# vfrantc/Bayesian-Enhancement-Model

Hardware: AMD Instinct MI355X
Metric: images/sec (whole node) CG_UNet N=8 Bayesian eval @256x256 (higher is better)
Workload: dtype f32

## Files before the change

bayesian-enhancement-model_amd/bem/modules.py:

```python
from __future__ import annotations

import math
from typing import Optional

import torch
import torch.nn as nn

from . import autograd as ag
from . import ops
from .bayes import BayesBank, Conv2dReparameterization, EvalSampleBank, Linear2dReparameterization, SampleCtx, sampling, set_module_paths
from .native import BemNativeError


def grad_mode(m: nn.Module) -> bool:
    return m.training and torch.is_grad_enabled()


def _need_cuda(x):
    if not x.is_cuda:
        raise BemNativeError("BEM modules run on the GPU through libbem_hip.so only (no CPU fallback); "
                             "move the model and input to a HIP device")


class LayerNorm2d(nn.LayerNorm):
# ... 131 lines not shown


class gdMlp(nn.Module):
    def __init__(self, in_features, hidden_features=None, out_features=None, act_layer=nn.GELU, drop=0.0, channels_first=False):
        super().__init__()
        out_features = out_features or in_features
        hidden_features = hidden_features or in_features
        self.project_in = PwConv2d(in_features, hidden_features * 2)
        self.dwconv = DwConv2d(hidden_features * 2)
        self.project_out = PwConv2d(hidden_features, out_features)
        self.act = act_layer()

    def fused_supported(self, C):
        return isinstance(self.project_in, PwConv2d) and isinstance(self.dwconv, DwConv2d) and isinstance(self.project_out, PwConv2d) \
            and ops.gdmlp_x6_supported(C, self.project_in.out_channels // 2)

    def forward_fused(self, x, norm: LayerNorm2d, pre=None):
        B, C = x.shape[0], x.shape[1]
        Hd = self.project_in.out_channels // 2
        if self.fused_supported(C):
            pi, dw, po = self.project_in, self.dwconv, self.project_out

            def prep():
                perm = ops.gate_interleave(Hd, pi.weight.device)
                bg = pi.bias.detach()[perm].contiguous() if pi.bias is not None else torch.zeros(2 * Hd, device=pi.weight.device)
                return (ops.pack_pw_weight(pi.weight.detach().reshape(2 * Hd, C)[perm].contiguous(), x6=True), bg,
                        ops.dw_gate_params10(dw.weight.detach(), None if dw.bias is None else dw.bias.detach(), Hd),
                        ops.pack_pw_weight(po.weight.detach().reshape(po.out_channels, Hd).contiguous(), x6=True),
                        None if po.bias is None else po.bias.detach().contiguous())
            Wg, bg, w10, Wo, bo = ops.derived(self).get("gdmlp_x6", [t for t in (pi.weight, pi.bias, dw.weight, dw.bias, po.weight, po.bias) if t is not None], prep)
            return ops.gdmlp_x6(x, norm.weight.detach(), norm.bias.detach(), norm.eps, Wg, bg, w10, Wo, bo, Hd, pre=pre)
        if pre is not None:
            raise BemNativeError("gdMlp: the SS2D tail can be folded into the one-kernel branch only")
        return self.chain(x, norm)[0]

    def chain(self, x, norm: LayerNorm2d):
        B = x.shape[0]
        t2 = ag.ln_pw(x, norm, self.project_in)
        w, b = self.dwconv.dw_weights(B)
        g = ops.dwconv3x3(t2, w, b, mode=2)
        Wp, b = self.project_out.gemm_weights(B)
        return ops.pw_gemm(g, Wp, ag.out_width(self.project_out), bias=b, res=x), t2, g


SS2D_MAX_D_STATE = 16


class SS2D(nn.Module):

    def __init__(self, d_model=96, d_state=16, ssm_ratio=2.0, dt_rank="auto", act_layer=nn.SiLU, d_conv=3,
                 conv_bias=True, dropout=0.0, bias=False, dt_min=0.001, dt_max=0.1, dt_init="random", dt_scale=1.0,
                 dt_init_floor=1e-4, initialize="v0", forward_type="v2", channel_first=False, **kwargs):
        super().__init__()
        if forward_type != "v05_noz" or not channel_first or d_conv != 3 or initialize != "v0":
            raise NotImplementedError("SS2D: only forward_type='v05_noz', channel_first, d_conv=3, init v0 are on the BEM path")
        N = int(d_state)
        if not 1 <= N <= SS2D_MAX_D_STATE:
            raise NotImplementedError(f"SS2D: d_state = {N}: the fused HIP scans take 1 <= d_state <= {SS2D_MAX_D_STATE}")
        d_inner = int(ssm_ratio * d_model)
        R = math.ceil(d_model / 16) if dt_rank == "auto" else dt_rank
        self.d_inner, self.dt_rank, self.d_state = d_inner, R, N
        self.in_proj = Linear2d(d_model, d_inner, bias=bias)
        self.act = act_layer()
        self.conv2d = DwConv2d(d_inner, bias=conv_bias)
        K = 4
        self.x_proj_weight = nn.Parameter(torch.stack([nn.Linear(d_inner, R + 2 * N, bias=False).weight.detach() for _ in range(K)], 0))
        self.out_proj = Linear2d(d_inner, d_model, bias=bias)
# ... 110 lines not shown
```

bayesian-enhancement-model_amd/bem/ops.py:

```python
from __future__ import annotations

import ctypes
import os
from inspect import signature as _signature
from functools import wraps as _wraps
from math import prod as _prod
from typing import Optional

import torch

from . import native
from .native import PwArgs, check, lib
from .tables import UIQM_WIDTH, lab_tables, niqe_gamma_table, niqe_resize_table, pil_resize_table, uiqm_resized_rows


_U64 = (1 << 64) - 1


def _stream():
    return ctypes.c_void_p(torch.cuda.current_stream().cuda_stream)


def _p(t: Optional[torch.Tensor]):
    return ctypes.c_void_p(0 if t is None else t.data_ptr())
# ... 575 lines not shown
    for n_, t in (("x", x), ("ln_w", ln_w), ("ln_b", ln_b), ("Wp_gate", Wp_gate), ("bias_gate", bias_gate), ("dw10", dw10), ("Wp_out", Wp_out)):
        _chk(t, n_)
    _chk(bias_out, "bias_out", optional=True)
    B, C, H, W = x.shape
    if not gdmlp_x6_supported(C, Hd):
        raise ValueError(f"gdmlp_x6: C = {C} (<= 80) / Hd = {Hd} (% 16) not supported")
    if tuple(dw10.shape) != (Hd, 10, 2):
        raise ValueError("gdmlp_x6: depthwise parameters must come from dw_gate_params10")
    if ln_w.numel() != C or ln_b.numel() != C or bias_gate.numel() != 2 * Hd or (bias_out is not None and bias_out.numel() != C):
        raise ValueError("gdmlp_x6: parameter shapes")
    _chk_packed1("gdmlp_x6", (("Wp_gate", Wp_gate, 2 * Hd, C), ("Wp_out", Wp_out, C, Hd)))
    _tile_plane_set("gdmlp_x6", C * H * W)
    if pre is not None:
        y0, y1, on_w, on_b, on_eps, Wp_op, b_op = pre
        for n_, t in (("y0", y0), ("y1", y1), ("on_w", on_w), ("on_b", on_b), ("Wp_outproj", Wp_op)):
            _chk(t, n_)
        _chk(b_op, "bias_outproj", optional=True)
        if not vss_back_supported(C, Hd, H * W):
            raise ValueError(f"gdmlp_x6 with pre: C = {C} (<= 48, % 8) with {C * H * W} elements per image (< {_TILE_NARROW}) not supported")
        if y0.shape != x.shape or y1.shape != x.shape or on_w.numel() != C or on_b.numel() != C or (b_op is not None and b_op.numel() != C):
            raise ValueError("gdmlp_x6 with pre: y0 / y1 must have the shape of x, out_norm and the out_proj bias C entries")
        _chk_packed1("gdmlp_x6", (("Wp_outproj", Wp_op, 32 * ((8 * ((C + 15) // 16) + 15) // 16), C),))
    out = torch.empty_like(x)
    if pre is not None:
        check(lib().bem_vss_back_x6_f32(_p(x), _p(ln_w), _p(ln_b), float(ln_eps), _p(Wp_gate), _p(bias_gate), _p(dw10), _p(Wp_out),
                                        _p(bias_out), _p(out), B, C, Hd, H, W, _p(y0), _p(y1), _p(on_w), _p(on_b), float(on_eps),
                                        _p(Wp_op), _p(b_op), _stream()), "gdmlp_x6")
        return out
    check(lib().bem_gdmlp_x6_f32(_p(x), _p(ln_w), _p(ln_b), float(ln_eps), _p(Wp_gate), _p(bias_gate), _p(dw10), _p(Wp_out),
                                 _p(bias_out), _p(out), B, C, Hd, H, W, _stream()), "gdmlp_x6")
    return out


def _dwconv3x3_cost(x, mode, **_):
    B, Cin, H, W = x.shape
    return 4.0 * B * H * W * (Cin + (Cin // 2 if mode == 2 else Cin)), 18.0 * B * Cin * H * W


@_bracket(_dwconv3x3_cost)
def dwconv3x3(x, w, bias=None, mode=0):
    _chk(x, "x"); _chk(w, "w"); _chk(bias, "bias", optional=True)
    B, Cin, H, W = x.shape
    Cout = Cin // 2 if mode == 2 else Cin
    per_b = w.dim() == 5
    Cw = w.shape[1] if per_b else w.shape[0]
    if Cw != Cin or tuple(w.shape[-3:]) != (1, 3, 3) or (per_b and w.shape[0] != B):
        raise ValueError(f"dwconv3x3: weight {tuple(w.shape)} vs input channels {Cin}")
    bb = 0
    if bias is not None:
        if bias.shape[-1] != Cin:
            raise ValueError("dwconv3x3: bias shape")
        bb = Cin if (bias.dim() == 2 and bias.shape[0] == B and B > 1) else 0
        if bias.dim() == 2 and bias.shape[0] not in (1, B):
            raise ValueError("dwconv3x3: bias batch")
    out = torch.empty(B, Cout, H, W, device=x.device, dtype=x.dtype)
    check(lib().bem_dwconv3x3_f32(_p(x), _p(w), (Cin * 9 if per_b else 0), _p(bias), bb, _p(out), B, Cout, H, W, mode,
                                  _stream()), "dwconv3x3")
    return out


USE_CONV_MFMA = True
USE_CONV_X6 = True


class ConvWeight:

    def __init__(self, w, input_grad=None):
        self.w, self._x6, self._f32, self._grad = w, None, None, input_grad

    def x6(self):
        if self._x6 is None:
            w = self.w
            self._x6 = pack_pw_weight(w.permute(2, 3, 0, 1).reshape(w.shape[2] * w.shape[3], w.shape[0], w.shape[1]).contiguous(), x6=True)
        return self._x6

    def f32(self):
        if self._f32 is None:
            self._f32 = pack_pw_weight(self.w.reshape(self.w.shape[0], -1).contiguous(), x6=False)
        return self._f32

    def input_grad(self):
        if self._grad is None:
            self._grad = ConvWeight(self.w.flip(2, 3).transpose(0, 1).contiguous())
        return self._grad


_CONV_FORMS = {1: ("rows", ConvWeight.x6), 2: ("taps", ConvWeight.x6), 3: ("mfma", ConvWeight.f32), 4: ("direct", lambda cw: cw.w)}
_CONV_ROUTES = {}


def _conv_out_hw(H, W, KH, KW, stride, pad, dilation=1):
    return (H + 2 * pad - dilation * (KH - 1) - 1) // stride + 1, (W + 2 * pad - dilation * (KW - 1) - 1) // stride + 1


def _conv2d_cost(x, w, stride, pad, res1, res2, dilation, **_):
# ... 12 lines not shown
    B, Ct, H, W = x.shape
    Cout, Cin, KH, KW = w.shape
    c0 = 0
    if cin_slice is not None:
        c0, cs = cin_slice
        if cs != Cin or c0 + Cin > Ct:
            raise ValueError("conv2d: channel slice out of range")
    elif Ct != Cin:
        raise ValueError(f"conv2d: input has {Ct} channels, weight expects {Cin}")
    if bias is not None and bias.shape != (Cout,):
        raise ValueError("conv2d: bias shape")
    if res1_rep < 1 or (res1_rep != 1 and res1 is None):
        raise ValueError("conv2d: res1_rep must be >= 1 and needs res1")
    oshape = (B, Cout) + _conv_out_hw(H, W, KH, KW, stride, pad, dilation)
    for n, r, shp in (("res1", res1, (B // res1_rep if B % res1_rep == 0 else -1,) + oshape[1:]), ("res2", res2, oshape)):
        if r is not None and tuple(r.shape) != shp:
            raise ValueError(f"conv2d: {n} shape")
    xs = _pslice(x, c0)
    key = (Cout, Cin, KH, KW, H, W, xs[1], stride, pad, dilation, USE_CONV_X6, USE_CONV_MFMA, (xs[0].value or 0) & 15,
           None if res1 is None else res1.data_ptr() & 15, None if res2 is None else res2.data_ptr() & 15)
    form = _CONV_ROUTES.get(key) or _CONV_ROUTES.setdefault(key, lib().bem_conv2d_route(
        *xs, _p(res1), _p(res2), None, Cin, H, W, Cout, KH, KW, stride, pad, dilation, USE_CONV_X6 | 2 * USE_CONV_MFMA))
    if form == 0:
        raise native.BemNativeError(lib().bem_last_error().decode())
    return form, cw, xs, oshape


def conv2d_route(x, w, stride=1, pad=1, res1=None, res2=None, cin_slice=None, dilation=1, res1_rep=1):
    return _CONV_FORMS[_conv2d_ask(x, w, None, stride, pad, res1, res2, cin_slice, dilation, res1_rep)[0]][0]


@_bracket(_conv2d_cost)
def conv2d(x, w, bias=None, stride=1, pad=1, relu=False, res1=None, res2=None, cin_slice=None, dilation=1, res1_rep=1):
    res1_rep = int(res1_rep)
    form, cw, xs, oshape = _conv2d_ask(x, w, bias, stride, pad, res1, res2, cin_slice, dilation, res1_rep)
    out = torch.empty(oshape, device=x.device, dtype=x.dtype)
    name, operand = _CONV_FORMS[form]
    (B, _, H, W), (Cout, Cin, KH, KW) = x.shape, cw.w.shape
    check(lib().bem_conv2d_f32(form, *xs, _p(operand(cw)), _p(bias), _p(res1), _p(res2), _p(out), B, Cin, H, W, Cout, KH, KW, stride, pad, dilation,
                               int(relu), res1_rep, _stream()), "conv2d " + name)
    return out


def quat_dwt(x, c0=0):
    _chk(x, "x")
    B, Ct, H, W = x.shape
    if c0 + 3 > Ct or H % 2 or W % 2:
        raise ValueError("quat_dwt: needs 3 channels and even H, W")
    out = torch.empty(B, 32, H // 2, W // 2, device=x.device, dtype=x.dtype)
    check(lib().bem_quat_dwt_f32(*_pslice(x, c0), _p(out), B, H, W, _stream()), "quat_dwt")
    return out


def cond_dwt(conds, s):
    _chk(conds, "conds")
    s = int(s)
    R, C, H, W = conds.shape
    if C != 3 or s < 1 or (H * s) % 2 or (W * s) % 2:
        raise ValueError("cond_dwt: needs 3 channels and even enlarged H, W")
    out = torch.empty(R, 32, H * s // 2, W * s // 2, device=conds.device, dtype=conds.dtype)
    check(lib().bem_cond_dwt_f32(_p(conds), _p(out), R, H, W, s, _stream()), "cond_dwt")
    return out


def dwt(x):
    _chk(x, "x")
    B, C, H, W = x.shape
# ... 1343 lines not shown
```

bayesian-enhancement-model_amd/csrc/gdmlp_x6.hip:

```cpp
#include "bem_common.h"
#include "x6_tile.h"

namespace {

struct GdX {
    const float* x; const float* ln_w; const float* ln_b; float ln_eps;
    const u32x4* Wpi;
    const u32x4* Wpo;
    const float* bgi;
    const float* dw10;
    int C, Hd, H, W, NCH, tx;
};

struct GdPre {
    const float* y0; const float* y1; const float* on_w; const float* on_b; float on_eps;
    const u32x4* Wop;
    const float* bop; float bopmul;
};

template <typename OFF>
__device__ __forceinline__ float at_byte(const float* base, OFF byte) {
    return *reinterpret_cast<const float*>(reinterpret_cast<const char*>(base) + byte);
}
template <typename OFF>
__device__ __forceinline__ void put_byte(float* base, OFF byte, float v) {
    *reinterpret_cast<float*>(reinterpret_cast<char*>(base) + byte) = v;
}

constexpr int GD_GS = 20;
constexpr bool GD_LO_PERSIST = true;

__device__ __forceinline__ float gelu_gate1(float a, float b) {
    const float t = __builtin_amdgcn_rcpf(fmaf(0.3275911f * 0.70710678118654752440f, fabsf(a), 1.f));
    float p = fmaf(1.061405429f, t, -1.453152027f);
    p = fmaf(p, t, 1.421413741f);
    p = fmaf(p, t, -0.284496736f);
    p = fmaf(p, t, 0.254829592f);
    const float e = __builtin_amdgcn_exp2f(a * a * -0.72134752044448170368f);
    const float r = fmaf(-(p * t), e, 1.f);
    const float h = 0.5f * a;
    return fmaf(h, copysignf(r, a), h) * b;
}

template <int KBM, int MTO, int WOB, bool PL2, bool PRE, typename OFF = uint32_t>
__device__ __forceinline__ void gdmlp_x6_tile(const GdX& k, const GdPre& pre, const float* __restrict__ bpo, float bomul, float* __restrict__ out) {
    constexpr int NPI = 3 * KBM, NPO = 3 * MTO;
    __shared__ __attribute__((aligned(16))) f32x2 T[16 * XT_TS];
    __shared__ __attribute__((aligned(16))) float G[128 * GD_GS];
    __shared__ __attribute__((aligned(16))) u32x4 Wis[2][NPI * 64];
    __shared__ __attribute__((aligned(16))) u32x4 Wos[WOB][NPO * 64];
    __shared__ __attribute__((aligned(16))) f32x2 Bss[2][16];
    __shared__ __attribute__((aligned(16))) f32x2 DWs[2][16 * 10];
    const int lane = threadIdx.x & 63, wave = __builtin_amdgcn_readfirstlane(threadIdx.x >> 6), kh = lane >> 5, n = lane & 31;
    const int b = blockIdx.z;
    int y0, x0;
    tile_origin(k.tx, y0, x0);
    const int L = k.H * k.W;
    const float* xb = k.x + (int64_t)b * k.C * L;

    const uint32_t voff = 16 * lane;
    const uint32_t wi_lds = lds_addr(Wis), wo_lds = lds_addr(Wos), bs_lds = lds_addr(Bss), dw_lds = lds_addr(DWs);
    auto dma_in = [&](int ji, int buf) {
#pragma unroll
        for (int t = 0; t < (NPI + 3) / 4; ++t) {
            const int p = wave + 4 * t;
            if (p < NPI) glds16(k.Wpi + ((int64_t)ji * NPI + p) * 64, voff, wi_lds + (buf * NPI + p) * 1024);
        }
        if (wave == (NPI & 3)) {
            const float* src = k.dw10 + (int64_t)ji * 320;
            glds16(src, voff, dw_lds + buf * 1280);
            if (lane < 16) glds16(src + 256, voff, dw_lds + buf * 1280 + 1024);
        }
        if (wave == ((NPI + 1) & 3) && lane < 8) glds16(k.bgi + (int64_t)ji * 32, voff, bs_lds + buf * 128);
    };
    auto dma_out = [&](int jo, int buf) {
// ... 487 lines not shown
```

include/bem_hip.h:

```cpp
#ifndef BEM_HIP_H
#define BEM_HIP_H

#include <stdint.h>

#ifdef __cplusplus
extern "C" {
#endif

#define BEM_OK 0
#define BEM_ERR_INVALID 1
#define BEM_ERR_LAUNCH 2

const char* bem_last_error(void);
int bem_abi_version(void);


int bem_selective_scan_fwd_f32(const float* u, const float* delta, const float* A, const float* Bm,
                               const float* Cm, const float* D, const float* delta_bias, float* out,
                               int batch, int dim, int L, int dstate, int ngroups, int delta_softplus,
                               void* stream);

int bem_selective_scan_fwd_in16(const void* u, const void* delta, const float* A, const void* Bm, const void* Cm, const float* D,
                                const float* delta_bias, float* out, int in_dtype, int batch, int dim, int L, int dstate,
                                int ngroups, int delta_softplus, void* stream);
// ... 40 lines not shown
    float* out; int out_mode; int Win;
    int B; int M; int K; int L;
} bem_pw_args;
int bem_pack_pw_weight_f32(const float* W, float* Wp, int nsets, int M, int K, void* stream);
int64_t bem_pw_packed_elems(int M, int K);

int bem_pw_gemm_x6_f32(const bem_pw_args* a, void* stream);
int bem_pack_pw_weight_x6(const float* W, float* Wp, int nsets, int M, int K, void* stream);
int bem_pack_pw_weight_x6_strided(const float* W, float* Wp, int nsets, int M, int K, int64_t set_stride, int64_t row_stride,
                                  int64_t col_stride, void* stream);
int bem_pack_pw_weight_x6_jobs(const void* jobs, const void* blks, int nblk, float* arena, void* stream);
int64_t bem_pw_x6_packed_elems(int M, int K);
int bem_bnn_sample_pack_x6(const float* mu, const float* rho, const float* eps, float* Wp, int nsets, int M, int K,
                           uint64_t seed, uint64_t stream_id, const uint64_t* stream_add, int sigma_given,
                           void* stream);
int bem_upfuse_x6_f32(const float* f, const float* skip, const float* Wc_packed, const float* Wf2_packed, const float* bias, float* out,
                      int B, int Cin, int h, int w, void* stream);

int bem_dwconv3x3_f32(const float* x, const float* w, int64_t w_bstride, const float* bias,
                      int64_t bias_bstride, float* out, int B, int Cout, int H, int W, int mode, void* stream);

#define BEM_CONV_ROWS 1
#define BEM_CONV_TAPS 2
#define BEM_CONV_MFMA 3
#define BEM_CONV_DIRECT 4
int bem_conv2d_f32(int form, const float* x, int64_t x_bstride, const float* w, const float* bias, const float* res1, const float* res2,
                   float* out, int B, int Cin, int H, int W, int Cout, int KH, int KW, int stride, int pad, int dilation, int relu,
                   int res1_rep, void* stream);

#define BEM_CONV_ALLOW_X6 1
#define BEM_CONV_ALLOW_MFMA 2
int bem_conv2d_route(const float* x, int64_t x_bstride, const float* res1, const float* res2, const float* out, int Cin, int H, int W,
                     int Cout, int KH, int KW, int stride, int pad, int dilation, int allow);

int bem_quat_dwt_f32(const float* rgb, int64_t x_bstride, float* out, int B, int H, int W, void* stream);
int bem_cond_dwt_f32(const float* cond, float* out, int R, int H, int W, int s, void* stream);
int bem_dwt_f32(const float* x, float* out, int B, int C, int H, int W, void* stream);
int bem_iwt_f32(const float* x, float* out, int B, int C4, int H, int W, void* stream);
int bem_iwt_hamilton_f32(const float* q1w, const float* q2w, float* out, int B, int h, int w, void* stream);
int bem_hamilton_f32(const float* q, float* out, int B, int H, int W, void* stream);

int bem_hamilton_full_f32(const float* q1, const float* q2, float* out, int B, int H, int W, void* stream);

int bem_attn_stats_f64(const float* f1, const float* f2, double* stats, int B, int L, void* stream);
int bem_attn_fold_f32(const double* stats, const float* attn_w ,
                      const float* fuse_w , const float* fuse_b ,
                      float* W_out , float* bias_out , int B, int L,
                      void* stream);
int bem_attn_fold_drop_f32(const double* stats, const float* attn_w, const float* fuse_w, const float* fuse_b,
                           const float* mask_or_null, float p, uint64_t seed, uint64_t stream_id,
                           float* W_out, float* bias_out, int B, int L, void* stream);

int bem_transpose_planes_f32(const float* src, int64_t src_bstride, float* dst, int64_t dst_bstride,
                             int nbatch, int ppb, int H, int W, void* stream);
int bem_copy_channels_f32(const float* src, int64_t src_bstride, float* dst, int64_t dst_bstride,
                          int B, int C, int L, void* stream);
int bem_copy_channels_rep_f32(const float* src, int64_t src_bstride, float* dst, int64_t dst_bstride, int B, int C, int L, int rep,
                              void* stream);
int bem_add_channels_f32(const float* src, int64_t src_bstride, float* dst, int64_t dst_bstride,
                         int B, int C, int L, void* stream);
int bem_bilinear_up_f32(const float* src, int64_t src_bstride, float* dst, int64_t dst_bstride,
                        int B, int C, int H, int W, int s, void* stream);
int bem_space_to_depth_f32(const float* x, float* out, int B, int C, int H, int W, void* stream);
int bem_pixel_shuffle2_f32(const float* x, float* out, int B, int C, int H, int W, void* stream);

int bem_bnn_ebank_sample_f32(const void* segs, const void* blks, int nblk, float* arena, uint64_t seed, uint64_t stream_base, void* stream);
// ... 22 lines not shown
int bem_candidate_finalize_f32(const float* pred, const float* target, float* final_out, float* psnr, double* ws,
                               int Bn, int samples_per_image, int Hp, int Wp, int h, int w, int gt_mean,
                               void* stream);

int bem_ssim_f32(const float* pred, const float* target, float* ssim, double* ws, int Bn, int samples_per_image, int h, int w, void* stream);

int bem_select_scores_f32(const float* cand, const float* s1, const float* s2, float weight, int rule, int* best, float* best_s1,
                          float* best_s2, float* best_img, int B, int N, int64_t chw, void* stream);

int bem_niqe_f32(const float* final, const double* mu_pris, const double* cov_pris, const double* window, const double* gam_tab, int ntab,
                 const float* rs_wh, const int* rs_ih, int kh, const float* rs_ww, const int* rs_iw, int kw, double* scores, void* ws,
                 int64_t ws_bytes, int Bn, int h, int w, void* stream);
int64_t bem_niqe_ws_bytes(int Bn, int h, int w);

int bem_uiqm_uciqe_f32(const float* final, const int* lab_tab, const int* rs_bh, const int* rs_kh, int kh, const int* rs_bv, const int* rs_kv,
                       int kv, double* uiqm, double* uciqe, void* ws, int64_t ws_bytes, int Bn, int h, int w, int Hr, void* stream);
int64_t bem_uiqm_ws_bytes(int Bn, int h, int w, int Hr);

int bem_mc_mean_f32(const float* pred, const float* target, float* out, double* ws, int B, int N, int Hp, int Wp, int h, int w,
                    int gt_mean, void* stream);

int bem_mc_accum_f32(const float* raw, const float* fin, float* sum, float* mean, float* m2, int B, int Nc, int n_done, int Hp, int Wp,
                     int h, int w, void* stream);

int bem_mc_finish_f32(const float* sum, const float* m2, const float* target, float* mc, float* std, double* std_mean, double* ws, int B,
                      int N, int h, int w, int gt_mean, void* stream);

int bem_select_merge_f32(const float* cand, const float* scores, int rule, int* best, float* best_score, float* best_img, int* pick, int B,
                         int Nc, int n_done, int64_t chw, void* stream);

int bem_gdmlp_x6_f32(const float* x, const float* ln_w, const float* ln_b, float ln_eps, const float* Wp_gate,
                     const float* bias_gate, const float* dw_gate10, const float* Wp_out,
                     const float* bias_out, float* out, int B, int C, int Hd, int H, int W, void* stream);

int bem_vss_back_x6_f32(const float* x, const float* ln_w, const float* ln_b, float ln_eps, const float* Wp_gate,
                        const float* bias_gate, const float* dw_gate10, const float* Wp_out,
                        const float* bias_out, float* out, int B, int C, int Hd, int H, int W,
                        const float* y0, const float* y1, const float* on_w, const float* on_b, float on_eps,
                        const float* Wp_outproj, const float* bias_outproj, void* stream);

int bem_ss2d_front_x6_f32(const float* x, const float* ln_w, const float* ln_b, float ln_eps, const float* Wp_in, const float* bias_in,
                          const float* dww, const float* dwb, const float* Wp_x, float* xc, float* xd, int B, int C, int Mx, int H, int W,
                          void* stream);


int bem_l1_loss_f32(const float* pred, const float* gt, float* dpred, float* loss, double* ws, int64_t n, float weight,
                    const float* gmul, void* stream);

int bem_ssim_loss_tile(void);
int64_t bem_ssim_loss_ws_elems(int64_t planes, int H, int W);
int bem_ssim_loss_f32(const float* pred, const float* gt, float* loss, float* coef, double* ws, int64_t planes, int H, int W,
                      float weight, void* stream);
int bem_ssim_loss_bwd_f32(const float* pred, const float* gt, const float* coef, float* dpred, int64_t planes, int H, int W,
                          float weight, const float* gmul, void* stream);

int bem_mse_loss_f32(const float* pred, const float* gt, float* dpred, float* loss, double* ws, int64_t n, float weight,
                     const float* gmul, void* stream);

int bem_pixstat_loss_chunk(void);
int64_t bem_pixstat_loss_ws_bytes(int64_t B, int64_t n1);
int bem_pixstat_loss_f32(const float* pred, const float* gt, float* out, double* rec, void* ws, int64_t B, int64_t n1, double a1,
                         double a3, double a5, double a6, void* stream);
int bem_pixstat_loss_bwd_f32(const float* pred, const float* gt, const double* rec, float* dpred, int64_t B, int64_t n1,
                             const float* gmul, void* stream);

int bem_iwt_hamilton_bwd_f32(const float* q1w, const float* q2w, const float* dout, float* dq1w, float* dq2w, int B, int h, int w,
// ... 124 lines not shown
```

bayesian-enhancement-model_amd/csrc/conv_x6.hip:

```cpp
#include "bem_common.h"
#include "conv_launch.h"
#include "scan_common.h"
#include "x6_common.h"

namespace {

struct CrX {
    const float* x; int64_t x_bs;
    const u32x4* Wp; const float* bias; const float* res1; const float* res2; float* out;
    int Cin, H, W, Ho, Wo, Cout, KB, MT, wo_shift, relu, mt_first, res1_rep;
};

typedef float f32x4v __attribute__((ext_vector_type(4)));

template <int MTW, int KS, int S>
__global__ __launch_bounds__(256, 2) void conv_rows_x6_kernel(CrX k) {
    constexpr int NPX = 4 / S;
    constexpr int NP = 3 * KS * MTW;
    __shared__ __attribute__((aligned(16))) u32x4 Ws[2][NP * 64];
    const int lane = threadIdx.x & 63, wave = __builtin_amdgcn_readfirstlane(threadIdx.x >> 6), kh = lane >> 5, n = lane & 31;
    const int b = blockIdx.z, mt0 = k.mt_first + blockIdx.y * MTW;
    const int Lo = k.Ho * k.Wo, Li = k.H * k.W;
    const int p0 = (xcd_tile(blockIdx.x, gridDim.x) * 4 + wave) * (32 * NPX);
    const int p = p0 + NPX * n;
    const bool live = p < Lo;
    const int pc = live ? p : 0;
    const int yo = pc >> k.wo_shift, xo = pc & (k.Wo - 1);
    const float lmask = xo == 0 ? 0.f : 1.f, rmask = xo == k.Wo - NPX ? 0.f : 1.f;
    const float* xb = k.x + (int64_t)b * k.x_bs;
    const uint32_t voff = 16 * lane, ws_lds = lds_addr(Ws);
    const int NS = KS * k.KB;

    auto dma_w = [&](int s, int buf) {
        const int kb = s / KS, r = s - kb * KS;
#pragma unroll
        for (int t = 0; t < (NP + 3) / 4; ++t) {
            const int pi = wave + 4 * t, kx = pi / (3 * MTW), m = (pi / 3) % MTW, li = pi % 3;
            if (pi < NP)
                glds16(k.Wp + ((((int64_t)(KS * r + kx) * k.MT + (mt0 + m)) * k.KB + kb) * 3 + li) * 64, voff, ws_lds + (buf * NP + pi) * 1024);
        }
    };
    auto load_x = [&](int s, f32x4v (&dst)[8], float& mk) {
        const int kb = min(s / KS, k.KB - 1), r = s - (s / KS) * KS;
// ... 42 lines not shown
                const u32x4* wp = Wc + (kx * MTW + m) * 192;
                const u32x4 wl[3] = {wp[0], wp[64], wp[128]};
#pragma unroll
                for (int j = 0; j < NPX; ++j) mac6(wl, xl[S * j + kx], acc[m][j], alo[m][j]);
            }
        asm volatile("s_waitcnt vmcnt(0)" ::: "memory");
        __syncthreads();
    }

    if (live) {
        typedef float fpx __attribute__((ext_vector_type(NPX)));
        const float lo = k.relu ? 0.f : -3.402823466e38f;
        const int64_t ob = (int64_t)b * k.Cout * Lo + pc;
        const float* r1b = k.res1 + (int64_t)(b / k.res1_rep) * k.Cout * Lo + pc;
#pragma unroll
        for (int m = 0; m < MTW; ++m)
#pragma unroll
            for (int r = 0; r < 16; ++r) {
                const int row = acc_row(r, kh, (mt0 + m) * 32);
                if (row < k.Cout) {
                    const float bv = k.bias ? k.bias[row] : 0.f;
                    const int64_t o = ob + (int64_t)row * Lo;
                    fpx v;
#pragma unroll
                    for (int j = 0; j < NPX; ++j) v[j] = fmaxf(acc[m][j][r] + alo[m][j][r] + bv, lo);
                    if (k.res1) v += *reinterpret_cast<const fpx*>(r1b + (int64_t)row * Lo);
                    if (k.res2) v += *reinterpret_cast<const fpx*>(k.res2 + o);
                    *reinterpret_cast<fpx*>(k.out + o) = v;
                }
            }
    }
}

}

bool conv_rows_shape(int KS, int Cin, int H, int W) {
    const int S = KS == 4 ? 2 : 1, Wo = W / S, lanes = Wo * S / 4;
    return Cin > 0 && Cin % 8 == 0 && H > 0 && H % S == 0 && W % S == 0 && lanes >= 1 && lanes <= 32 && (Wo & (Wo - 1)) == 0;
}
bool conv_rows_aligned(const float* x, int64_t x_bstride, const float* out, const float* res1, const float* res2) {
    return (((uintptr_t)x | (uintptr_t)out | (uintptr_t)res1 | (uintptr_t)res2) & 15) == 0 && x_bstride % 4 == 0;
}

int conv_rows_launch(int KS, const float* x, int64_t x_bstride, const float* Wp, const float* bias, const float* res1, const float* res2, float* out,
                     int B, int Cin, int H, int W, int Cout, int relu, int res1_rep, void* stream) {
    const char* what = KS == 4 ? "conv4x4s2_x6" : "conv3x3_x6";
    BEM_REQUIRE(x && Wp && out, "%s: null tensor", what);
    BEM_REQUIRE(res1_rep >= 1, "%s: res1_rep %d", what, res1_rep);
    BEM_REQUIRE(B >= 0 && B <= 65535 && Cout > 0 && (KS == 3 || KS == 4) && conv_rows_shape(KS, Cin, H, W), "%s: shape outside the row form", what);
    BEM_REQUIRE(((uintptr_t)Wp & 15) == 0 && conv_rows_aligned(x, x_bstride, out, res1, res2), "%s: alignment (x, packed weights, out and residuals 16 bytes)", what);
    const int S = KS == 4 ? 2 : 1, Ho = H / S, Wo = W / S;
    BEM_REQUIRE((int64_t)Cout * Ho * Wo < (1ll << 30) && (int64_t)Cin * H * W < (1ll << 30), "%s: plane set too large for 32-bit lane offsets", what);
    if (B == 0) return BEM_OK;
    CrX k;
    k.x = x; k.x_bs = x_bstride; k.Wp = reinterpret_cast<const u32x4*>(Wp); k.bias = bias; k.res1 = res1; k.res2 = res2; k.out = out;
    k.Cin = Cin; k.H = H; k.W = W; k.Ho = Ho; k.Wo = Wo; k.Cout = Cout; k.KB = cdiv(Cin, 16); k.MT = cdiv(Cout, 32); k.relu = relu; k.res1_rep = res1_rep;
    k.wo_shift = __builtin_ctz(Wo);
    hipStream_t s = (hipStream_t)stream;
    if (KS == 4) {
        const int pairs = k.MT / 2, nx = cdiv(Ho * Wo, 256);
        if (pairs) {
            k.mt_first = 0;
            conv_rows_x6_kernel<2, 4, 2><<<dim3(nx, pairs, B), 256, 0, s>>>(k);
        }
        if (k.MT & 1) {
            k.mt_first = 2 * pairs;
            conv_rows_x6_kernel<1, 4, 2><<<dim3(nx, 1, B), 256, 0, s>>>(k);
        }
    } else {
        k.mt_first = 0;
        conv_rows_x6_kernel<1, 3, 1><<<dim3(cdiv(Ho * Wo, 512), k.MT, B), 256, 0, s>>>(k);
    }
    return bem_check_launch(what);
}

namespace {

struct CvX {
    const float* x; int64_t x_bs;
    const u32x4* Wp; const float* bias; const float* res1; const float* res2; float* out;
    int Cin, H, W, Ho, Wo, Cout, KB, MT, relu, pad, dil, res1_rep;
};

template <int MTW, int KH, int KW, int S>
__global__ __launch_bounds__(256, 2) void conv_taps_x6_kernel(CvX k) {
    constexpr int NSUB = 2, NTAP = KH * KW;
    const int lane = threadIdx.x & 63, wave = threadIdx.x >> 6, kh = lane >> 5, n = lane & 31;
    const int b = blockIdx.z, mt0 = blockIdx.y * MTW;
    const int Lo = k.Ho * k.Wo, Li = k.H * k.W;
    const int p0 = (xcd_tile(blockIdx.x, gridDim.x) * 4 + wave) * 64;
    if (p0 >= Lo) return;
    const int p = p0 + 2 * n;
    const bool live = p < Lo;
    const int pc = live ? p : 0;
    const int yo = pc / k.Wo, xo = pc - yo * k.Wo;
    const int yi0 = yo * S - k.pad, xi0 = xo * S - k.pad;
    const float* xb = k.x + (int64_t)b * k.x_bs;
    f32x16 acc[MTW][NSUB], alo[MTW][NSUB];
#pragma unroll
for (int m = 0; m < MTW; ++m)
#pragma unroll
// ... 133 lines not shown
```

Measured before the change: 362.2.

## Fuse depthwise gate and output projection into one gdMlp back kernel

Adds a new HIP kernel that fuses the depthwise 3x3 conv, GELU gating, output pointwise projection, bias and residual add for gdMlp blocks where the single-kernel x6 path does not apply (larger C up to 160). The input projection with LayerNorm still runs as a separate pw_gemm, but the gated intermediate no longer goes through global memory and one launch is dropped. The kernel double-buffers weights and depthwise parameters in LDS. It adds a new code path with its own tiling and register pressure, which could underperform the previous dwconv+gemm chain for some shapes.

```diff
diff --git a/bayesian-enhancement-model_amd/bem/modules.py b/bayesian-enhancement-model_amd/bem/modules.py
--- a/bayesian-enhancement-model_amd/bem/modules.py
+++ b/bayesian-enhancement-model_amd/bem/modules.py
@@ -187,7 +187,25 @@
             return ops.gdmlp_x6(x, norm.weight.detach(), norm.bias.detach(), norm.eps, Wg, bg, w10, Wo, bo, Hd, pre=pre)
         if pre is not None:
             raise BemNativeError("gdMlp: the SS2D tail can be folded into the one-kernel branch only")
+        if ops.USE_GDMLP_BACK and self.back_supported(x):
+            pi, dw, po = self.project_in, self.dwconv, self.project_out
+
+            def prep():
+                perm = ops.gate_interleave(Hd, pi.weight.device)
+                return (ops.pack_pw_weight(pi.weight.detach().reshape(2 * Hd, C)[perm].contiguous(), x6=True),
+                        None if pi.bias is None else pi.bias.detach()[perm].contiguous(),
+                        ops.dw_gate_params10(dw.weight.detach(), None if dw.bias is None else dw.bias.detach(), Hd),
+                        ops.pack_pw_weight(po.weight.detach().reshape(po.out_channels, Hd).contiguous(), x6=True),
+                        None if po.bias is None else po.bias.detach().contiguous())
+            Wg, bg, w10, Wo, bo = ops.derived(self).get("gdmlp_back", [t for t in (pi.weight, pi.bias, dw.weight, dw.bias, po.weight, po.bias) if t is not None], prep)
+            t2 = ops.pw_gemm(x, Wg, 2 * Hd, ln=(norm.weight.detach(), norm.bias.detach()), ln_eps=norm.eps, bias=bg)
+            return ops.gdmlp_back(x, t2, w10, Wo, bo, Hd)
         return self.chain(x, norm)[0]
+
+    def back_supported(self, x):
+        return type(self.project_in) is PwConv2d and type(self.dwconv) is DwConv2d and type(self.project_out) is PwConv2d \
+            and not grad_mode(self) and self.project_out.out_channels == x.shape[1] \
+            and ops.gdmlp_back_supported(x.shape[1], self.project_in.out_channels // 2, x.shape[2] * x.shape[3])
 
     def chain(self, x, norm: LayerNorm2d):
         B = x.shape[0]
diff --git a/bayesian-enhancement-model_amd/bem/ops.py b/bayesian-enhancement-model_amd/bem/ops.py
--- a/bayesian-enhancement-model_amd/bem/ops.py
+++ b/bayesian-enhancement-model_amd/bem/ops.py
@@ -631,6 +631,39 @@
     return out
 
 
+USE_GDMLP_BACK = True
+
+
+def gdmlp_back_supported(C, Hd, L):
+    return C <= 160 and Hd % 16 == 0 and C * L < _TILE_NARROW and L < (1 << 27)
+
+
+def _gdmlp_back_cost(x, t2, Hd, **_):
+    return 4.0 * (t2.numel() + 2 * x.numel()), 6.0 * 2.0 * x.numel() * Hd
+
+
+@_bracket(_gdmlp_back_cost)
+def gdmlp_back(x, t2, dw10, Wp_out, bias_out, Hd):
+    for n_, t in (("x", x), ("t2", t2), ("dw10", dw10), ("Wp_out", Wp_out)):
+        _chk(t, n_)
+    _chk(bias_out, "bias_out", optional=True)
+    if x.dim() != 4:
+        raise ValueError("gdmlp_back: x must be (B, C, H, W)")
+    B, C, H, W = x.shape
+    if not gdmlp_back_supported(C, Hd, H * W):
+        raise ValueError(f"gdmlp_back: C = {C} (<= 160) / Hd = {Hd} (% 16) with {H * W} pixels per plane ({C * H * W} < {_TILE_NARROW}) not supported")
+    if tuple(t2.shape) != (B, 2 * Hd, H, W):
+        raise ValueError(f"gdmlp_back: t2 shape {tuple(t2.shape)} != {(B, 2 * Hd, H, W)}")
+    if tuple(dw10.shape) != (Hd, 10, 2):
+        raise ValueError("gdmlp_back: depthwise parameters must come from dw_gate_params10")
+    if bias_out is not None and bias_out.numel() != C:
+        raise ValueError("gdmlp_back: parameter shapes")
+    _chk_packed1("gdmlp_back", (("Wp_out", Wp_out, C, Hd),))
+    out = torch.empty_like(x)
+    check(lib().bem_gdmlp_back_x6_f32(_p(x), _p(t2), _p(dw10), _p(Wp_out), _p(bias_out), _p(out), B, C, Hd, H, W, _stream()), "gdmlp_back")
+    return out
+
+
 def _dwconv3x3_cost(x, mode, **_):
     B, Cin, H, W = x.shape
     return 4.0 * B * H * W * (Cin + (Cin // 2 if mode == 2 else Cin)), 18.0 * B * Cin * H * W
diff --git a/bayesian-enhancement-model_amd/csrc/gdmlp_back_x6.hip b/bayesian-enhancement-model_amd/csrc/gdmlp_back_x6.hip
--- /dev/null
+++ b/bayesian-enhancement-model_amd/csrc/gdmlp_back_x6.hip
@@ -0,0 +1,223 @@
+#include "bem_common.h"
+#include "gdmlp_gate.h"
+
+namespace {
+
+struct GbX {
+    const float* x;
+    const float* t2;
+    const u32x4* Wpo;
+    const float* dw10;
+    const float* bpo; float bomul;
+    int C, Hd, H, W, NCH, tx, tiles;
+};
+
+template <int MTO>
+__global__ __launch_bounds__(256, 2) void gdmlp_back_x6_kernel(GbX k, float* __restrict__ out) {
+    constexpr int NPO = 3 * MTO;
+    __shared__ __attribute__((aligned(16))) f32x2 T[16 * XT_TS];
+    __shared__ __attribute__((aligned(16))) float G[128 * GD_GS];
+    __shared__ __attribute__((aligned(16))) u32x4 Wos[2][NPO * 64];
+    __shared__ __attribute__((aligned(16))) f32x2 DWs[2][16 * 10];
+    const int lane = threadIdx.x & 63, wave = __builtin_amdgcn_readfirstlane(threadIdx.x >> 6), kh = lane >> 5, n = lane & 31;
+    const int t = xcd_tile(blockIdx.x, gridDim.x);
+    const int b = t / k.tiles, tile = t - b * k.tiles, tyi = tile / k.tx;
+    const int y0 = tyi * XT_TH, x0 = (tile - tyi * k.tx) * XT_TW;
+    const int L = k.H * k.W;
+    const uint32_t L4 = 4u * (uint32_t)L;
+    const float* const xb = k.x + (int64_t)b * k.C * L;
+    const float* const t2b = k.t2 + (int64_t)b * (2 * k.Hd) * L;
+
+    const uint32_t voff = 16 * lane;
+    const uint32_t wo_lds = lds_addr(Wos), dw_lds = lds_addr(DWs);
+    auto dma_dw = [&](int ji, int buf) {
+        if (wave == (NPO & 3)) {
+            const float* src = k.dw10 + (int64_t)ji * 320;
+            glds16(src, voff, dw_lds + buf * 1280);
+            if (lane < 16) glds16(src + 256, voff, dw_lds + buf * 1280 + 1024);
+        }
+    };
+    auto dma_out = [&](int jo, int buf) {
+#pragma unroll
+        for (int i = 0; i < (NPO + 3) / 4; ++i) {
+            const int p = wave + 4 * i, mt = p / 3, li = p - 3 * mt;
+            if (p < NPO) glds16(k.Wpo + (((int64_t)mt * k.NCH + jo) * 3 + li) * 64, voff, wo_lds + (buf * NPO + p) * 1024);
+        }
+    };
+    dma_dw(0, 0);
+
+    uint32_t toff[4], tbit[4];
+#pragma unroll
+    for (int i = 0; i < 4; ++i) {
+        const int hp = min(lane + 64 * i, XT_NPH - 1);
+        const int hy = hp / XT_HW, hx = hp - hy * XT_HW;
+        const int gy = y0 - 1 + hy, gx = x0 - 1 + hx;
+        tbit[i] = gy >= 0 && gy < k.H && gx >= 0 && gx < k.W ? 0xffffffffu : 0u;
+        toff[i] = 4u * (uint32_t)(min(max(gy, 0), k.H - 1) * k.W + min(max(gx, 0), k.W - 1));
+    }
+    float tv[4][8];
+    auto t_load = [&](int jc) {
+        const float* const base = t2b + (int64_t)(32 * jc + 8 * wave) * L;
+#pragma unroll
+        for (int i = 0; i < 4; ++i)
+#pragma unroll
+            for (int q = 0; q < 8; ++q) tv[i][q] = at_byte(base, toff[i] + (uint32_t)q * L4);
+    };
+    auto t_store = [&]() {
+#pragma unroll
+        for (int i = 0; i < 4; ++i)
+            if (i < 3 || lane < XT_NPH - 192) {
+#pragma unroll
+                for (int cc = 0; cc < 4; ++cc)
+                    T[(4 * wave + cc) * XT_TS + lane + 64 * i] =
+                        f32x2{bitsf(fbits(tv[i][2 * cc]) & tbit[i]), bitsf(fbits(tv[i][2 * cc + 1]) & tbit[i])};
+            }
+    };
+    t_load(0);
+
+    const int wb_lds = 2 * kh * XT_HW + n;
+    const int c_lo = 4 * wave;
+
+    constexpr bool LOP = MTO <= 2;
+    f32x16 oh[MTO], ol[MTO];
+#pragma unroll
+    for (int mt = 0; mt < MTO; ++mt)
+#pragma unroll
+        for (int r = 0; r < 16; ++r) {
+            oh[mt][r] = 0.f;
+            if (LOP) ol[mt][r] = 0.f;
+        }
+
+    auto phase_c = [&](const u32x4* Wo) {
+        const float* gp = G + (wave * 32 + n) * GD_GS + 8 * kh;
+        const f32x4 ga = *reinterpret_cast<const f32x4*>(gp), gb = *reinterpret_cast<const f32x4*>(gp + 4);
+        const float v[8] = {ga[0], ga[1], ga[2], ga[3], gb[0], gb[1], gb[2], gb[3]};
+        u32x4 gl[3];
+        split8(v, gl[0], gl[1], gl[2]);
+#pragma unroll
+        for (int mt = 0; mt < MTO; ++mt) {
+            const u32x4* wp = Wo + mt * 192 + lane;
+            const u32x4 wl[3] = {wp[0], wp[64], wp[128]};
+            if constexpr (LOP) mac6(wl, gl, oh[mt], ol[mt]);
+            else {
+                f32x16 lo;
+#pragma unroll
+                for (int r = 0; r < 16; ++r) lo[r] = 0.f;
+                mac6(wl, gl, oh[mt], lo);
+                oh[mt] += lo;
+            }
+        }
+    };
+
+    asm volatile("s_waitcnt vmcnt(0)" ::: "memory");
+    __syncthreads();
+
+#pragma clang loop unroll(disable)
+    for (int j = 0; j < k.NCH; ++j) {
+        const int cur = j & 1;
+        if (j + 1 < k.NCH) dma_dw(j + 1, cur ^ 1);
+        dma_out(j, cur);
+        t_store();
+        __builtin_amdgcn_sched_barrier(0);
+        if (j + 1 < k.NCH) t_load(j + 1);
+        if (j) phase_c(Wos[cur ^ 1]);
+        __syncthreads();
+        {
+            f32x2 g[4];
+#pragma unroll
+            for (int cc = 0; cc < 4; ++cc) {
+                const f32x4* wv = reinterpret_cast<const f32x4*>(DWs[cur] + (c_lo + cc) * 10);
+                const f32x4 w01 = wv[0], w23 = wv[1], w45 = wv[2], w67 = wv[3], w8b = wv[4];
+                const f32x2 wq[9] = {{w01[0], w01[1]}, {w01[2], w01[3]}, {w23[0], w23[1]}, {w23[2], w23[3]}, {w45[0], w45[1]},
+                                     {w45[2], w45[3]}, {w67[0], w67[1]}, {w67[2], w67[3]}, {w8b[0], w8b[1]}};
+                const f32x2 bias = {w8b[2], w8b[3]};
+                const f32x2* tp = T + (c_lo + cc) * XT_TS + wb_lds;
+                f32x2 win[4][3];
+#pragma unroll
+                for (int dy = 0; dy < 4; ++dy)
+#pragma unroll
+                    for (int dx = 0; dx < 3; ++dx) win[dy][dx] = tp[dy * XT_HW + dx];
+                float a0x = bias[0], a0y = bias[1], a1x = bias[0], a1y = bias[1];
+#pragma unroll
+                for (int ty = 0; ty < 3; ++ty)
+#pragma unroll
+                    for (int tx = 0; tx < 3; ++tx) {
+                        const f32x2 w = wq[3 * ty + tx], u0 = win[ty][tx], u1 = win[ty + 1][tx];
+                        a0x = fmaf(w[0], u0[0], a0x); a0y = fmaf(w[1], u0[1], a0y);
+                        a1x = fmaf(w[0], u1[0], a1x); a1y = fmaf(w[1], u1[1], a1y);
+                    }
+                g[cc] = f32x2{gelu_gate1(a0x, a0y), gelu_gate1(a1x, a1y)};
+            }
+#pragma unroll
+            for (int p = 0; p < 2; ++p)
+                *reinterpret_cast<f32x4*>(G + ((2 * kh + p) * 32 + n) * GD_GS + c_lo) = f32x4{g[0][p], g[1][p], g[2][p], g[3][p]};
+        }
+        asm volatile("s_waitcnt vmcnt(0)" ::: "memory");
+        __syncthreads();
+    }
+    phase_c(Wos[(k.NCH - 1) & 1]);
+    __builtin_amdgcn_sched_barrier(0);
+
+    const int oy = y0 + wave, ox = x0 + n;
+    const bool opix = oy < k.H && ox < k.W;
+    const uint32_t pix4 = 4u * (uint32_t)(min(oy, k.H - 1) * k.W + min(ox, k.W - 1));
+    float* const ob = out + (int64_t)b * k.C * L;
+    const uint32_t po4 = pix4 + (uint32_t)(4 * kh) * L4;
+    float rs[2][16];
+    auto load_res = [&](int mt) {
+#pragma unroll
+        for (int r = 0; r < 16; ++r) {
+            const int ru = acc_row(r, 0, 32 * mt);
+            if (mt < MTO - 1) rs[mt & 1][r] = fmaf(valu_copy(at_byte(k.bpo + ru, (uint32_t)(16 * kh))), k.bomul, at_byte(xb + (int64_t)ru * L, po4));
+            else {
+                const int rc = min(ru + 4 * kh, k.C - 1);
+                rs[mt & 1][r] = fmaf(valu_copy(k.bpo[rc]), k.bomul, at_byte(xb, pix4 + (uint32_t)rc * L4));
+            }
+        }
+    };
+    load_res(0);
+#pragma unroll
+    for (int mt = 0; mt < MTO; ++mt) {
+        __builtin_amdgcn_sched_barrier(0);
+        if (mt + 1 < MTO) load_res(mt + 1);
+        if (opix) {
+#pragma unroll
+            for (int r = 0; r < 16; ++r) {
+                const int ru = acc_row(r, 0, 32 * mt);
+                const float v = (LOP ? oh[mt][r] + ol[mt][r] : oh[mt][r]) + rs[mt & 1][r];
+                if (mt < MTO - 1 || ru + 4 * kh < k.C) put_byte(ob + (int64_t)ru * L, po4, v);
+            }
+        }
+    }
+}
+
+}
+
+extern "C" int bem_gdmlp_back_x6_f32(const float* x, const float* t2, const float* dw_gate10, const float* Wp_out, const float* bias_out,
+                                     float* out, int B, int C, int Hd, int H, int W, void* stream) {
+    const char* op = "gdmlp_back_x6";
+    BEM_REQUIRE(x && t2 && dw_gate10 && Wp_out && out, "%s: null tensor", op);
+    BEM_REQUIRE(B >= 0 && C > 0 && C <= 160 && Hd > 0 && Hd % 16 == 0 && H > 0 && W > 0,
+                "%s: needs C <= 160 and Hd %% 16 == 0 (got C = %d, Hd = %d)", op, C, Hd);
+    BEM_REQUIRE((((uintptr_t)Wp_out | (uintptr_t)dw_gate10) & 15) == 0, "%s: packed weights and depthwise parameters must be 16-byte aligned", op);
+    BEM_REQUIRE(x != out && t2 != out, "%s: in-place operation is not supported (halo reads)", op);
+    BEM_REQUIRE((int64_t)C * H * W < (1ll << 30) && (int64_t)H * W < (1ll << 27), "%s: plane set too large for 32-bit byte offsets", op);
+    GbX k;
+    k.x = x; k.t2 = t2; k.Wpo = reinterpret_cast<const u32x4*>(Wp_out); k.dw10 = dw_gate10;
+    k.bpo = bias_out ? bias_out : dw_gate10;
+    k.bomul = bias_out ? 1.f : 0.f;
+    k.C = C; k.Hd = Hd; k.H = H; k.W = W; k.NCH = Hd / 16; k.tx = cdiv(W, XT_TW); k.tiles = k.tx * cdiv(H, XT_TH);
+    const int64_t nwg = (int64_t)k.tiles * B;
+    BEM_REQUIRE(nwg < (1ll << 31), "%s: too many tiles for one grid (%lld)", op, (long long)nwg);
+    if (B == 0) return BEM_OK;
+    const dim3 grid((unsigned)nwg);
+    hipStream_t s = (hipStream_t)stream;
+    switch (cdiv(C, 32)) {
+        case 1: gdmlp_back_x6_kernel<1><<<grid, 256, 0, s>>>(k, out); break;
+        case 2: gdmlp_back_x6_kernel<2><<<grid, 256, 0, s>>>(k, out); break;
+        case 3: gdmlp_back_x6_kernel<3><<<grid, 256, 0, s>>>(k, out); break;
+        case 4: gdmlp_back_x6_kernel<4><<<grid, 256, 0, s>>>(k, out); break;
+        default: gdmlp_back_x6_kernel<5><<<grid, 256, 0, s>>>(k, out); break;
+    }
+    return bem_check_launch(op);
+}
diff --git a/bayesian-enhancement-model_amd/csrc/gdmlp_gate.h b/bayesian-enhancement-model_amd/csrc/gdmlp_gate.h
--- /dev/null
+++ b/bayesian-enhancement-model_amd/csrc/gdmlp_gate.h
@@ -0,0 +1,29 @@
+#pragma once
+#include "x6_tile.h"
+
+namespace {
+
+template <typename OFF>
+__device__ __forceinline__ float at_byte(const float* base, OFF byte) {
+    return *reinterpret_cast<const float*>(reinterpret_cast<const char*>(base) + byte);
+}
+template <typename OFF>
+__device__ __forceinline__ void put_byte(float* base, OFF byte, float v) {
+    *reinterpret_cast<float*>(reinterpret_cast<char*>(base) + byte) = v;
+}
+
+constexpr int GD_GS = 20;
+
+__device__ __forceinline__ float gelu_gate1(float a, float b) {
+    const float t = __builtin_amdgcn_rcpf(fmaf(0.3275911f * 0.70710678118654752440f, fabsf(a), 1.f));
+    float p = fmaf(1.061405429f, t, -1.453152027f);
+    p = fmaf(p, t, 1.421413741f);
+    p = fmaf(p, t, -0.284496736f);
+    p = fmaf(p, t, 0.254829592f);
+    const float e = __builtin_amdgcn_exp2f(a * a * -0.72134752044448170368f);
+    const float r = fmaf(-(p * t), e, 1.f);
+    const float h = 0.5f * a;
+    return fmaf(h, copysignf(r, a), h) * b;
+}
+
+}
diff --git a/bayesian-enhancement-model_amd/csrc/gdmlp_x6.hip b/bayesian-enhancement-model_amd/csrc/gdmlp_x6.hip
--- a/bayesian-enhancement-model_amd/csrc/gdmlp_x6.hip
+++ b/bayesian-enhancement-model_amd/csrc/gdmlp_x6.hip
@@ -1,5 +1,5 @@
 #include "bem_common.h"
-#include "x6_tile.h"
+#include "gdmlp_gate.h"
 
 namespace {
 
@@ -18,29 +18,7 @@
     const float* bop; float bopmul;
 };
 
-template <typename OFF>
-__device__ __forceinline__ float at_byte(const float* base, OFF byte) {
-    return *reinterpret_cast<const float*>(reinterpret_cast<const char*>(base) + byte);
-}
-template <typename OFF>
-__device__ __forceinline__ void put_byte(float* base, OFF byte, float v) {
-    *reinterpret_cast<float*>(reinterpret_cast<char*>(base) + byte) = v;
-}
-
-constexpr int GD_GS = 20;
 constexpr bool GD_LO_PERSIST = true;
-
-__device__ __forceinline__ float gelu_gate1(float a, float b) {
-    const float t = __builtin_amdgcn_rcpf(fmaf(0.3275911f * 0.70710678118654752440f, fabsf(a), 1.f));
-    float p = fmaf(1.061405429f, t, -1.453152027f);
-    p = fmaf(p, t, 1.421413741f);
-    p = fmaf(p, t, -0.284496736f);
-    p = fmaf(p, t, 0.254829592f);
-    const float e = __builtin_amdgcn_exp2f(a * a * -0.72134752044448170368f);
-    const float r = fmaf(-(p * t), e, 1.f);
-    const float h = 0.5f * a;
-    return fmaf(h, copysignf(r, a), h) * b;
-}
 
 template <int KBM, int MTO, int WOB, bool PL2, bool PRE, typename OFF = uint32_t>
 __device__ __forceinline__ void gdmlp_x6_tile(const GdX& k, const GdPre& pre, const float* __restrict__ bpo, float bomul, float* __restrict__ out) {
diff --git a/include/bem_hip.h b/include/bem_hip.h
--- a/include/bem_hip.h
+++ b/include/bem_hip.h
@@ -184,6 +184,9 @@
 int bem_gdmlp_x6_f32(const float* x, const float* ln_w, const float* ln_b, float ln_eps, const float* Wp_gate,
                      const float* bias_gate, const float* dw_gate10, const float* Wp_out,
                      const float* bias_out, float* out, int B, int C, int Hd, int H, int W, void* stream);
+
+int bem_gdmlp_back_x6_f32(const float* x, const float* t2, const float* dw_gate10, const float* Wp_out, const float* bias_out,
+                          float* out, int B, int C, int Hd, int H, int W, void* stream);
 
 int bem_vss_back_x6_f32(const float* x, const float* ln_w, const float* ln_b, float ln_eps, const float* Wp_gate,
                         const float* bias_gate, const float* dw_gate10, const float* Wp_out,
```

Result: no change. 364.4 (median of 6 runs) (+0.6%).

## Add LDS-tiled 3x3 conv kernel with resident weights for small channel counts

Applied to the files above, without the earlier changes.

Adds a new 3x3 conv path that stages all packed weights in LDS once per block and loads 2D spatial input tiles with halos into LDS. Each block then walks several tiles (tpw), prefetching the next input block into registers while the current one runs through the MFMA taps. The goal is to avoid re-reading weights and overlapping input rows in the row kernel for small Cin/Cout layers and small grids. The cost is extra __syncthreads per channel block and a large dynamic LDS allocation, which may lower occupancy. A runtime toggle is exposed to Python.

```diff
diff --git a/bayesian-enhancement-model_amd/bem/ops.py b/bayesian-enhancement-model_amd/bem/ops.py
--- a/bayesian-enhancement-model_amd/bem/ops.py
+++ b/bayesian-enhancement-model_amd/bem/ops.py
@@ -660,6 +660,12 @@
 
 USE_CONV_MFMA = True
 USE_CONV_X6 = True
+USE_CONV_TILE = True
+_conv_tile_set = True
+
+
+def conv_tile_supported(B, Cin, H, W, Cout):
+    return bool(lib().bem_conv_tile_shape(B, Cin, H, W, Cout))
 
 
 class ConvWeight:
@@ -738,7 +744,11 @@
 
 @_bracket(_conv2d_cost)
 def conv2d(x, w, bias=None, stride=1, pad=1, relu=False, res1=None, res2=None, cin_slice=None, dilation=1, res1_rep=1):
+    global _conv_tile_set
     res1_rep = int(res1_rep)
+    if USE_CONV_TILE != _conv_tile_set:
+        lib().bem_conv_tile_enable(int(USE_CONV_TILE))
+        _conv_tile_set = USE_CONV_TILE
     form, cw, xs, oshape = _conv2d_ask(x, w, bias, stride, pad, res1, res2, cin_slice, dilation, res1_rep)
     out = torch.empty(oshape, device=x.device, dtype=x.dtype)
     name, operand = _CONV_FORMS[form]
diff --git a/bayesian-enhancement-model_amd/csrc/conv_x6.hip b/bayesian-enhancement-model_amd/csrc/conv_x6.hip
--- a/bayesian-enhancement-model_amd/csrc/conv_x6.hip
+++ b/bayesian-enhancement-model_amd/csrc/conv_x6.hip
@@ -1,14 +1,14 @@
 #include "bem_common.h"
 #include "conv_launch.h"
 #include "scan_common.h"
-#include "x6_common.h"
+#include "x6_tile.h"
 
 namespace {
 
 struct CrX {
     const float* x; int64_t x_bs;
     const u32x4* Wp; const float* bias; const float* res1; const float* res2; float* out;
-    int Cin, H, W, Ho, Wo, Cout, KB, MT, wo_shift, relu, mt_first, res1_rep;
+    int Cin, H, W, Ho, Wo, Cout, KB, MT, wo_shift, relu, mt_first, res1_rep, tpw;
 };
 
 typedef float f32x4v __attribute__((ext_vector_type(4)));
@@ -117,6 +117,142 @@
     }
 }
 
+template <int KB, int MT>
+__global__ __launch_bounds__(256, 2) void conv_tile_x6_kernel(CrX k) {
+    extern __shared__ __attribute__((aligned(16))) u32x4 ct_lds[];
+    constexpr int NPW = 27 * KB * MT;
+    u32x4* const Ws = ct_lds;
+    u32x4* const Xs = ct_lds + NPW * 64;
+    const int lane = threadIdx.x & 63, wave = __builtin_amdgcn_readfirstlane(threadIdx.x >> 6), kh = lane >> 5, n = lane & 31;
+    const int b = blockIdx.z, Li = k.H * k.W;
+    const int tx = k.W >> 5, nti = tx * ((k.H + XT_TH - 1) / XT_TH);
+    const int t0 = xcd_tile(blockIdx.x, gridDim.x) * k.tpw, t1 = min(t0 + k.tpw, nti);
+    const float* xb = k.x + (int64_t)b * k.x_bs;
+    {
+        const uint32_t voff = 16 * lane, ws_lds = lds_addr(Ws);
+        for (int pi = wave; pi < NPW; pi += 4) {
+            const int li = pi % 3, m = (pi / 3) % MT, tap = (pi / (3 * MT)) % 9, kb = pi / (27 * MT);
+            glds16(k.Wp + (((int64_t)(tap * MT + m) * KB + kb) * 3 + li) * 64, voff, ws_lds + pi * 1024);
+        }
+    }
+    int hp[2], hy[2], hx[2];
+#pragma unroll
+    for (int i = 0; i < 2; ++i) {
+        hp[i] = (wave + 4 * i) * 32 + n;
+        hy[i] = hp[i] / XT_HW;
+        hx[i] = hp[i] - hy[i] * XT_HW;
+    }
+    const bool two = wave + 4 < XT_NPB;
+    auto load_x = [&](int tile, int kb, float (&dst)[2][8], float (&mk)[2]) {
+        const int tyi = tile / tx, y0 = tyi * XT_TH, x0 = (tile - tyi * tx) * XT_TW;
+#pragma unroll
+        for (int i = 0; i < 2; ++i)
+            if (i == 0 || two) {
+                const int gy = y0 - 1 + hy[i], gx = x0 - 1 + hx[i];
+                mk[i] = (hp[i] < XT_NPH && gy >= 0 && gy < k.H && gx >= 0 && gx < k.W) ? 1.f : 0.f;
+                const int off = min(max(gy, 0), k.H - 1) * k.W + min(max(gx, 0), k.W - 1);
+#pragma unroll
+                for (int e = 0; e < 8; ++e) dst[i][e] = xb[min(16 * kb + 8 * kh + e, k.Cin - 1) * Li + off];
+            }
+    };
+    auto stage_x = [&](const float (&src)[2][8], const float (&mk)[2]) {
+#pragma unroll
+        for (int i = 0; i < 2; ++i)
+            if (i == 0 || two) {
+                float v[8];
+#pragma unroll
+                for (int e = 0; e < 8; ++e) v[e] = src[i][e] * mk[i];
+                u32x4 l0, l1, l2;
+                split8(v, l0, l1, l2);
+                if (hp[i] < XT_NPH) {
+                    u32x4* xp = Xs + kh * XT_TS + hp[i];
+                    xp[0] = l0;
+                    xp[2 * XT_TS] = l1;
+                    xp[4 * XT_TS] = l2;
+                }
+            }
+    };
+
+    f32x16 acc[MT], alo[MT];
+#pragma unroll
+    for (int m = 0; m < MT; ++m) acc[m] = alo[m] = zero16();
+    float* const Bs = reinterpret_cast<float*>(Xs + 3 * 2 * XT_TS);
+    if (threadIdx.x < 32 * MT) Bs[threadIdx.x] = k.bias && (int)threadIdx.x < k.Cout ? k.bias[threadIdx.x] : 0.f;
+    float xn[2][8], mkn[2];
+    if (t0 < t1) load_x(t0, 0, xn, mkn);
+    asm volatile("s_waitcnt vmcnt(0)" ::: "memory");
+
+    const u32x4* Xw = Xs + kh * XT_TS + wave * XT_HW + n;
+    const float lo = k.relu ? 0.f : -3.402823466e38f;
+    for (int tile = t0; tile < t1; ++tile) {
+#pragma unroll
+        for (int kb = 0; kb < KB; ++kb) {
+            stage_x(xn, mkn);
+            __syncthreads();
+            if (kb + 1 < KB) load_x(tile, kb + 1, xn, mkn);
+            else if (tile + 1 < t1) load_x(tile + 1, 0, xn, mkn);
+#pragma unroll
+            for (int ky = 0; ky < 3; ++ky)
+#pragma unroll
+                for (int kx = 0; kx < 3; ++kx) {
+                    const u32x4* xp = Xw + ky * XT_HW + kx;
+                    const u32x4 xl[3] = {xp[0], xp[2 * XT_TS], xp[4 * XT_TS]};
+#pragma unroll
+                    for (int m = 0; m < MT; ++m) {
+                        const u32x4* wp = Ws + ((kb * 9 + 3 * ky + kx) * MT + m) * 192 + lane;
+                        const u32x4 wl[3] = {wp[0], wp[64], wp[128]};
+                        mac6(wl, xl, acc[m], alo[m]);
+                    }
+                }
+            __syncthreads();
+        }
+        const int tyi = tile / tx, oy = tyi * XT_TH + wave;
+        if (oy < k.H) {
+            const int pc = oy * k.W + (tile - tyi * tx) * XT_TW + n;
+            float* ob = k.out + (int64_t)b * k.Cout * Li + pc;
+            const float* r1b = k.res1 + (int64_t)(b / k.res1_rep) * k.Cout * Li + pc;
+            const float* r2b = k.res2 + (int64_t)b * k.Cout * Li + pc;
+#pragma unroll
+            for (int m = 0; m < MT; ++m) {
+                float v[16], q[16];
+#pragma unroll
+                for (int r = 0; r < 16; ++r) v[r] = fmaxf(acc[m][r] + alo[m][r] + Bs[acc_row(r, kh, m * 32)], lo);
+                if (k.res1) {
+#pragma unroll
+                    for (int r = 0; r < 16; ++r) q[r] = r1b[min(acc_row(r, kh, m * 32), k.Cout - 1) * Li];
+#pragma unroll
+                    for (int r = 0; r < 16; ++r) v[r] += q[r];
+                }
+                if (k.res2) {
+#pragma unroll
+                    for (int r = 0; r < 16; ++r) q[r] = r2b[min(acc_row(r, kh, m * 32), k.Cout - 1) * Li];
+#pragma unroll
+                    for (int r = 0; r < 16; ++r) v[r] += q[r];
+                }
+#pragma unroll
+                for (int r = 0; r < 16; ++r) {
+                    const int row = acc_row(r, kh, m * 32);
+                    if (row < k.Cout) ob[row * Li] = v[r];
+                }
+            }
+        }
+#pragma unroll
+        for (int m = 0; m < MT; ++m) acc[m] = alo[m] = zero16();
+    }
+}
+
+}
+
+static bool conv_tile_shape(int B, int Cin, int H, int W, int Cout) {
+    if (!(conv_rows_shape(3, Cin, H, W) && W % XT_TW == 0 && B > 0 && Cout > 0 && cdiv(Cin, 16) * cdiv(Cout, 32) <= 2)) return false;
+    return Cin <= 16 || (int64_t)B * (W / XT_TW) * cdiv(H, XT_TH) < 4096;
+}
+static bool conv_tile_on = true;
+extern "C" int bem_conv_tile_shape(int B, int Cin, int H, int W, int Cout) { return conv_tile_shape(B, Cin, H, W, Cout); }
+extern "C" int bem_conv_tile_enable(int on) {
+    const int was = conv_tile_on;
+    conv_tile_on = on != 0;
+    return was;
 }
 
 bool conv_rows_shape(int KS, int Cin, int H, int W) {
@@ -152,6 +288,17 @@
             k.mt_first = 2 * pairs;
             conv_rows_x6_kernel<1, 4, 2><<<dim3(nx, 1, B), 256, 0, s>>>(k);
         }
+    } else if (conv_tile_on && conv_tile_shape(B, Cin, H, W, Cout)) {
+        const int nti = (W / XT_TW) * cdiv(H, XT_TH);
+        const int64_t all = (int64_t)nti * B;
+        k.tpw = all >= 8192 ? 8 : all >= 4096 ? 4 : all >= 1024 ? 2 : 1;
+        const dim3 grid(cdiv(nti, k.tpw), 1, B);
+        const int lds = (27 * k.KB * k.MT * 64 + 3 * 2 * XT_TS) * 16 + 32 * k.MT * 4;
+#define BEM_CT(KBV, MTV) do { set_max_dynamic_lds<conv_tile_x6_kernel<KBV, MTV>>(lds); conv_tile_x6_kernel<KBV, MTV><<<grid, 256, lds, s>>>(k); } while (0)
+        if (k.KB == 2) BEM_CT(2, 1);
+        else if (k.MT == 2) BEM_CT(1, 2);
+        else BEM_CT(1, 1);
+#undef BEM_CT
     } else {
         k.mt_first = 0;
         conv_rows_x6_kernel<1, 3, 1><<<dim3(cdiv(Ho * Wo, 512), k.MT, B), 256, 0, s>>>(k);
diff --git a/include/bem_hip.h b/include/bem_hip.h
--- a/include/bem_hip.h
+++ b/include/bem_hip.h
@@ -96,6 +96,8 @@
 #define BEM_CONV_ALLOW_MFMA 2
 int bem_conv2d_route(const float* x, int64_t x_bstride, const float* res1, const float* res2, const float* out, int Cin, int H, int W,
                      int Cout, int KH, int KW, int stride, int pad, int dilation, int allow);
+int bem_conv_tile_shape(int B, int Cin, int H, int W, int Cout);
+int bem_conv_tile_enable(int on);
 
 int bem_quat_dwt_f32(const float* rgb, int64_t x_bstride, float* out, int B, int H, int W, void* stream);
 int bem_cond_dwt_f32(const float* cond, float* out, int R, int H, int W, int s, void* stream);
```

New measurement: 358.1 before, 359.0 after (median of 6 runs). About the same (+0.2%).
